# tayloraswift/swift-png

Measured on NVIDIA H100. Metric: MPixels/s decode (inflate+unfilter), higher is better.
Workload: dtype u8

## Files before the change

### swift-png_b200/csrc/inflate_wave.cuh

```cuda
#pragma once

#include "inflate_serial.cuh"

namespace pngb200 {

#ifndef WV_CTAS
#define WV_CTAS 2
#endif
constexpr int      WV_THREADS      = 256;
constexpr int      WV_CTAS_PER_SM  = WV_CTAS;
constexpr int      WV_WARPS        = WV_THREADS / 32;
constexpr uint32_t WV_SUB_BITS     = 256;
constexpr uint32_t WV_BITS         = WV_THREADS * WV_SUB_BITS;
constexpr uint32_t WV_WORDS        = WV_BITS / 32 + 8;
constexpr uint32_t WV_SMEM_WORDS   = WV_WORDS + WV_WORDS / 8 + 1;
constexpr uint32_t WV_RING         = 65536;
constexpr uint32_t WV_WINDOW       = 32768;
constexpr uint32_t WV_OUT_BYTES    = WV_RING - WV_WINDOW;
constexpr uint32_t WV_BITMAP_WORDS = WV_OUT_BYTES / 32;
constexpr uint32_t WV_LIST_CAP     = WV_BITS / 2 + 64;
constexpr uint64_t WV_MAX_WAVE_OUT = (uint64_t)WV_LIST_CAP * 258;
constexpr uint32_t WV_HDR_WORDS    = 192;
constexpr uint32_t ADLER_MOD32     = 65521;
#ifndef WV_POLL_NS
#define WV_POLL_NS 20
#endif
constexpr uint32_t WV_WALK_K       = 8;

#if defined(PNGB200_EMU) && defined(WV_PROFILE)
struct WvProfile { uint64_t thread_iters[8], warp_iters[8]; };
inline WvProfile& wv_profile() { static WvProfile p; return p; }
inline void wv_count(int phase, uint32_t iters)
{
    uint32_t m = iters;
    for (int o = 16; o; o >>= 1) m = max(m, __shfl_xor_sync(0xffffffffu, m, o));
    wv_profile().thread_iters[phase] += iters;
    if ((threadIdx.x & 31) == 0) wv_profile().warp_iters[phase] += m;
}
#define WV_COUNT(phase, iters) wv_count(phase, iters)
#else
#define WV_COUNT(phase, iters)
#endif

enum : uint32_t { PF_EOB = 1, PF_BAD = 2 };
enum : uint32_t { WK_SYNC = 0, WK_END = 1, WK_EOB = 2, WK_BAD = 3, WK_OWN_EOB = 4, WK_OWN_BAD = 5, WK_RUNNING = 6 };

struct WvHeader {
    int32_t  status, type, final, nlit, ndist;
    uint32_t stored;
    uint64_t pos;
};

struct WvShared {
    SerialShared ser;
    uint32_t     words[WV_SMEM_WORDS];
    uint32_t     mask[8 * WV_THREADS];
    uint32_t     ck[8 * WV_THREADS];
    uint32_t     exit_[WV_THREADS];
    uint32_t     wpos_[WV_THREADS];
    uint32_t     wn_[WV_THREADS];
    uint64_t     cross_[WV_THREADS];
    uint16_t     wc_[WV_THREADS];
    uint16_t     next_[WV_THREADS];
    uint8_t      kind_[WV_THREADS];
    uint8_t      wlist[2][WV_THREADS];
    uint16_t     dpre_[WV_THREADS];
    uint16_t     cst_[WV_THREADS];
    uint32_t     dsum[WV_WARPS];
    uint32_t     wcount[3];
    uint32_t     bitmap[WV_BITMAP_WORDS];
    uint8_t      ring[WV_RING] __align__(16);
    uint64_t     warp_sums[WV_WARPS + 1];
    uint32_t     adler_a[WV_WARPS], adler_b[WV_WARPS];
    uint32_t     exc[WV_WARPS], valid[WV_WARPS];
    uint32_t     mark[WV_WARPS];
    uint32_t     last, term, anomaly, ticket;
    uint64_t     cyc[12], tick;
    uint64_t     pf_bar;
    WvHeader     hdr;
};

struct WvParams {
    const StreamJob* jobs;
    StreamResult*    results;
    const uint32_t*  order;
    uint32_t*        ticket;
    uint8_t*         scratch;
    uint64_t         scratch_stride;
    uint64_t         bitmap_words;
    int              count;
    SwitchRecord*    switched = nullptr;
};

struct CopyItem { uint32_t o; uint32_t run_dist; };

#ifdef PNGB200_EMU
typedef uintptr_t saddr_t;
inline uint32_t lds32(saddr_t addr) { return *(const uint32_t*)addr; }
inline uint32_t bfe32(uint32_t x, uint32_t pos, uint32_t len);
inline saddr_t smem_addr(const void* p) { return (uintptr_t)p; }
inline saddr_t opaque(saddr_t a) { return a; }
inline uint32_t bmsk(uint32_t pos, uint32_t width)
{
    pos &= 0xff; width &= 0xff;
    if (pos > 31 || width == 0) return 0;
    const uint32_t m = width >= 32 ? ~0u : (1u << width) - 1u;
    return m << pos;
}
inline uint32_t bfe32(uint32_t x, uint32_t pos, uint32_t len) { return pos > 31 ? 0 : (x >> pos) & bmsk(0, len); }
#else
typedef uint32_t saddr_t;
__device__ __forceinline__ uint32_t lds32(uint32_t addr)
{
    uint32_t v;
    asm volatile("ld.shared.u32 %0, [%1];" : "=r"(v) : "r"(addr) : "memory");
    return v;
}
__device__ __forceinline__ uint32_t bmsk(uint32_t pos, uint32_t width)
{
    uint32_t r;
    asm("bmsk.clamp.b32 %0, %1, %2;" : "=r"(r) : "r"(pos), "r"(width));
    return r;
}
__device__ __forceinline__ uint32_t bfe32(uint32_t x, uint32_t pos, uint32_t len)
{
    return (x >> pos) & bmsk(0, len);
}
__device__ __forceinline__ uint32_t smem_addr(const void* p) { return (uint32_t)__cvta_generic_to_shared(p); }
__device__ __forceinline__ uint32_t opaque(uint32_t a)
{
    asm volatile("" : "+r"(a));
    return a;
}
#endif

#ifdef PNGB200_EMU
inline void mbar_init(uint64_t*, uint32_t) {}
inline void mbar_expect_tx(uint64_t*, uint32_t) {}
inline void bulk_g2s(void* dst, const void* src, uint32_t bytes, uint64_t*) { memcpy(dst, src, bytes); }
inline bool mbar_try_wait(uint64_t*, uint32_t) { return true; }
inline void fence_proxy_async() {}
inline void bulk_prefetch_l2(const void*, uint32_t) {}
#else
__device__ __forceinline__ void mbar_init(uint64_t* bar, uint32_t count)
{
    asm volatile("mbarrier.init.shared::cta.b64 [%0], %1;" ::"r"((uint32_t)__cvta_generic_to_shared(bar)), "r"(count) : "memory");
}
__device__ __forceinline__ void mbar_expect_tx(uint64_t* bar, uint32_t bytes)
{
    asm volatile("mbarrier.arrive.expect_tx.shared::cta.b64 _, [%0], %1;" ::"r"((uint32_t)__cvta_generic_to_shared(bar)), "r"(bytes) : "memory");
}
__device__ __forceinline__ void bulk_g2s(void* dst, const void* src, uint32_t bytes, uint64_t* bar)
{
    asm volatile("cp.async.bulk.shared::cluster.global.mbarrier::complete_tx::bytes [%0], [%1], %2, [%3];" ::"r"(
                     (uint32_t)__cvta_generic_to_shared(dst)),
                 "l"(src), "r"(bytes), "r"((uint32_t)__cvta_generic_to_shared(bar))
                 : "memory");
}
__device__ __forceinline__ bool mbar_try_wait(uint64_t* bar, uint32_t parity)
{
    uint32_t ok;
    asm volatile("{\n\t.reg .pred p;\n\tmbarrier.try_wait.parity.shared::cta.b64 p, [%1], %2;\n\tselp.u32 %0, 1, 0, p;\n\t}"
                 : "=r"(ok)
                 : "r"((uint32_t)__cvta_generic_to_shared(bar)), "r"(parity)
                 : "memory");
    return ok != 0;
}
__device__ __forceinline__ void fence_proxy_async() { asm volatile("fence.proxy.async.shared::cta;" ::: "memory"); }
__device__ __forceinline__ void bulk_prefetch_l2(const void* src, uint32_t bytes)
{
    asm volatile("cp.async.bulk.prefetch.L2.global [%0], %1;" ::"l"(src), "r"(bytes) : "memory");
}
#endif
constexpr uint32_t WV_PF_WORDS = WV_WORDS + 4;

struct FastBits {
    saddr_t  wbase;
    uint32_t wi;
    uint32_t cur, nxt;
    uint32_t off;
    uint32_t pos;
    __device__ __forceinline__ void init(saddr_t words_addr, uint32_t start)
    {
        wbase = words_addr;
        const uint32_t W = start >> 5;
        cur = lds32(wbase + ((W + (W >> 3)) << 2));
        nxt = lds32(wbase + ((W + 1 + ((W + 1) >> 3)) << 2));
        wi  = W + 2;
        off = start & 31;
        pos = start;
    }
    __device__ __forceinline__ uint32_t peek() const { return __funnelshift_r(cur, nxt, off); }
    __device__ __forceinline__ void skip(uint32_t n)
    {
        off += n;
        pos += n;
        if (off >= 32) {
            cur = nxt;
            nxt = lds32(wbase + ((wi + (wi >> 3)) << 2));
            ++wi;
            off -= 32;
        }
    }
};

template <int ROOT>
__device__ __forceinline__ uint32_t fast_lookup(saddr_t table_addr, uint32_t bits)
{
    uint32_t e = lds32(table_addr + ((bits & ((1u << ROOT) - 1u)) << 2));
    if ((e & (E_SPECIAL | E_PTR | E_INVALID)) == (E_SPECIAL | E_PTR))
        e = lds32(table_addr + (((e >> 16) + bfe32(bits, ROOT, e_skip(e) - ROOT)) << 2));
    return e;
}

template <bool WANT_DIST>
__device__ __forceinline__ uint32_t wv_decode(FastBits& b, saddr_t lit, saddr_t dst, uint32_t& run, uint32_t& dist,
                                              uint32_t& is_copy)
{
    const uint32_t bits = b.peek();
    const uint32_t e = fast_lookup<LIT_ROOT>(lit, bits);
    if (e & E_SPECIAL) {
        if (e & E_INVALID) return PF_BAD;
        b.skip(e_len(e));
        return PF_EOB;
    }
    const uint32_t len = e & 15u, skipn = (e >> 4) & 31u;
    run = (e >> 16) + bfe32(bits, len, skipn - len);
    b.skip(skipn);
    is_copy = (e >> 9) & 1u;
    const uint32_t dbits = b.peek();
    const uint32_t d = fast_lookup<DIST_ROOT>(dst, dbits);
    if (is_copy && (d & E_SPECIAL)) return PF_BAD;
    const uint32_t dlen = d & 15u, dskip = (d >> 4) & 31u;
    if (WANT_DIST) dist = (d >> 16) + bfe32(dbits, dlen, dskip - dlen);
    b.skip(is_copy ? dskip : 0u);
    return 0;
}

struct StagedReader {
    const uint32_t* w;
    uint64_t        base_bit, total_bits, pos;
    uint32_t        wi;
    uint64_t        buf;
    int             cnt;
    __device__ void init(const uint32_t* words, uint64_t base, uint64_t total, uint64_t p)
    {
        w = words; base_bit = base; total_bits = total;
        seek(p);
    }
    __device__ void seek(uint64_t p)
    {
        pos = p;
        wi  = (uint32_t)((p - base_bit) >> 5);
        buf = 0;
        cnt = 0;
        refill();
        int skip = (int)(p & 31);
        buf >>= skip;
        cnt -= skip;
    }
    __device__ __forceinline__ void refill()
    {
        while (cnt <= 32) {
            buf |= (uint64_t)(wi < WV_HDR_WORDS ? w[wi] : 0u) << cnt;
            cnt += 32;
            ++wi;
        }
    }
    __device__ __forceinline__ uint32_t peek() const { return (uint32_t)buf; }
    __device__ __forceinline__ void consume(int n) { buf >>= n; cnt -= n; pos += n; }
    __device__ __forceinline__ uint32_t take(int n)
    {
        uint32_t v = (uint32_t)buf & (n >= 32 ? ~0u : ((1u << n) - 1u));
        consume(n);
        return v;
    }
    __device__ __forceinline__ bool have(uint64_t n) const { return pos + n <= total_bits; }
};

__device__ __forceinline__ uint32_t bit_mask(uint32_t lo, uint32_t hi)
{
    return (hi >= 32 ? ~0u : ((1u << hi) - 1u)) & ~((1u << lo) - 1u);
}
__device__ __forceinline__ void bits_set(uint32_t* U, uint32_t o, uint32_t run)
{
    const uint32_t a = o & 31u;
    uint32_t*      w = U + (o >> 5);
    if (a + run <= 32u) { atomicOr(w, bmsk(a, run)); return; }
    atomicOr(w, ~0u << a);
    uint32_t rem = run - (32u - a);
    for (++w; rem >= 32u; ++w, rem -= 32u) atomicOr(w, ~0u);
    if (rem) atomicOr(w, bmsk(0, rem));
}
__device__ __forceinline__ void bits_clear(uint32_t* U, uint32_t o, uint32_t run)
{
    const uint32_t a = o & 31u;
    uint32_t*      w = U + (o >> 5);
    if (a + run <= 32u) { atomicAnd(w, ~bmsk(a, run)); return; }
    atomicAnd(w, ~(~0u << a));
    uint32_t rem = run - (32u - a);
    for (++w; rem >= 32u; ++w, rem -= 32u) atomicAnd(w, 0u);
    if (rem) atomicAnd(w, ~bmsk(0, rem));
}
__device__ __forceinline__ bool bits_all_clear(const uint32_t* U, uint32_t o, uint32_t run)
{
    const volatile uint32_t* w = U + (o >> 5);
    const uint32_t a = o & 31u;
    uint32_t any;
    if (a + run <= 32u) any = *w & bmsk(a, run);
    else {
        any = *w & (~0u << a);
        uint32_t rem = run - (32u - a);
        for (++w; rem >= 32u; ++w, rem -= 32u) any |= *w;
        if (rem) any |= *w & bmsk(0, rem);
    }
    __threadfence_block();
    return any == 0;
}

__device__ __forceinline__ void ring_copy(uint8_t* ring, uint32_t d, uint32_t s, uint32_t run, uint32_t dist)
{
    d &= 0xffffu;
    s &= 0xffffu;
    if (dist >= 4 && max(d, s) + run + 3 < WV_RING) {
        const uint8_t* sp = ring + s;
        uint8_t*       dp = ring + d;
        for (uint32_t k = 0; k < run; k += 4) {
            const uint8_t b0 = sp[k], b1 = sp[k + 1], b2 = sp[k + 2], b3 = sp[k + 3];
            dp[k] = b0;
            if (k + 1 < run) dp[k + 1] = b1;
            if (k + 2 < run) dp[k + 2] = b2;
            if (k + 3 < run) dp[k + 3] = b3;
        }
    } else {
        for (uint32_t k = 0; k < run; ++k) ring[(d + k) & 0xffffu] = ring[(s + k) & 0xffffu];
    }
}

template <typename T>
__device__ __forceinline__ void hbm_copy(T* hbm, uint32_t o, uint32_t run, uint32_t dist)
{
    T*       to   = hbm + o;
    const T* from = to - dist;
    if (dist >= 4) {
        uint32_t k = 0;
        for (; k + 4 <= run; k += 4) {
            const T b0 = from[k], b1 = from[k + 1], b2 = from[k + 2], b3 = from[k + 3];
            to[k] = b0; to[k + 1] = b1; to[k + 2] = b2; to[k + 3] = b3;
        }
        for (; k < run; ++k) to[k] = from[k];
    } else {
        uint32_t q = 0;
        for (uint32_t k = 0; k < run; ++k) {
            to[k] = from[q];
            if (++q == dist) q = 0;
        }
    }
}

struct EmitState {
    uint8_t*  ring;
    uint32_t  rbase;
    uint8_t*  hbm;
    uint32_t* U;
    CopyItem* list;
    uint32_t  reach;
    uint32_t  o;
    uint32_t  first;
    uint32_t  clean;
    uint32_t  c_next;
    bool      bad_ref;
};

template <bool IN_HBM>
__device__ __forceinline__ void emit_token(EmitState& S, uint32_t run, uint32_t dist, uint32_t is_copy)
{
    const uint32_t o = S.o;
    if (!is_copy) {
        if (IN_HBM) S.hbm[o] = (uint8_t)run;
        else S.ring[(S.rbase + o) & 0xffffu] = (uint8_t)run;
        S.o = o + 1;
        return;
    }
    if (dist > S.reach + o) {
        S.bad_ref = true;
        return;
    }
    const int32_t src = (int32_t)o - (int32_t)dist;
    bool final = src + (int32_t)run <= 0 || src >= (int32_t)S.clean;
    if (!final && src >= (int32_t)S.first)
        final = bits_all_clear(S.U, (uint32_t)src, min(run, dist));
    if (final) {
        if (IN_HBM) hbm_copy(S.hbm, o, run, dist);
        else ring_copy(S.ring, S.rbase + o, S.rbase + o - dist, run, dist);
    } else {
        bits_set(S.U, o, run);
        S.list[S.c_next++] = CopyItem{o, run | (dist - 1) << 16};
        S.clean = o + run;
    }
    S.o = o + run;
}

__device__ __forceinline__ void emit_token_sym(EmitState& S, uint32_t run, uint32_t dist, uint32_t is_copy)
{
    uint16_t* const h = reinterpret_cast<uint16_t*>(S.hbm);
    uint32_t o = S.o;
    if (!is_copy) {
        h[o] = (uint16_t)run;
        S.o = o + 1;
        return;
    }
    const uint32_t have = S.reach + o;
    if (dist > have) {
        const uint32_t pre = min(dist - have, run);
        const uint32_t idx = WV_WINDOW - (dist - have);
        for (uint32_t k = 0; k < pre; ++k) h[o + k] = (uint16_t)(0x8000u | (idx + k));
        o += pre;
        run -= pre;
        if (run == 0) { S.o = o; return; }
    }
    const int32_t src = (int32_t)o - (int32_t)dist;
    bool final = src + (int32_t)run <= 0 || src >= (int32_t)S.clean;
    if (!final && src >= (int32_t)S.first) final = bits_all_clear(S.U, (uint32_t)src, min(run, dist));
    if (final) {
        hbm_copy(h, o, run, dist);
    } else {
        bits_set(S.U, o, run);
        S.list[S.c_next++] = CopyItem{o, run | (dist - 1) << 16};
        S.clean = o + run;
    }
    S.o = o + run;
}

template <class Shared>
__device__ bool wv_fast_header(Shared& sh, uint64_t hbase_bit, uint64_t pos, uint64_t total_bits, int lane, WvHeader& out)
{
    const uint32_t* const W = sh.words;
    auto get = [&](uint32_t rel, uint32_t n) -> uint32_t {
        const uint32_t w = rel >> 5;
        const uint32_t v = __funnelshift_r(W[w], W[w + 1], rel & 31u);
        return n >= 32 ? v : v & ((1u << n) - 1u);
    };
    uint32_t rel = (uint32_t)(pos - hbase_bit);
    if (pos + 3 > total_bits) return false;
    const uint32_t h3 = get(rel, 3);
    rel += 3;
    out.status = PNGB200_OK;
    out.final = (int32_t)(h3 & 1u);
    out.type = (int32_t)(h3 >> 1);
    out.stored = 0;
    out.nlit = out.ndist = 0;
    if (out.type == 3) return false;
    if (out.type == 0) {
        const uint64_t boundary = (pos + 3 + 7) & ~(uint64_t)7;
        if (boundary + 32 > total_bits) return false;
        const uint32_t v = get((uint32_t)(boundary - hbase_bit), 32);
        const uint32_t l = v & 0xffffu, m = v >> 16;
        if (l != (~m & 0xffffu)) return false;
        out.stored = l;
        out.pos = boundary + 32;
        return true;
    }
    uint8_t* const lens = sh.ser.lens;
    if (out.type == 1) {
        for (int k = lane; k < 320; k += 32) lens[k] = k < 144 ? 8 : k < 256 ? 9 : k < 280 ? 7 : k < 288 ? 8 : 5;
        out.nlit = 288;
        out.ndist = 32;
        out.pos = pos + 3;
        __syncwarp();
        return true;
    }
    if (pos + 17 > total_bits) return false;
    const uint32_t v = get(rel, 14);
    rel += 14;
    const int nlit = 257 + (int)(v & 31u), ndist = 1 + (int)((v >> 5) & 31u), nclen = 4 + (int)(v >> 10);
    if (nlit > 286) return false;
    if (lane < 19) lens[lane] = 0;
    __syncwarp();
    if (lane < nclen) lens[c_clen_order[lane]] = (uint8_t)get(rel + 3u * (uint32_t)lane, 3);
    rel += 3u * (uint32_t)nclen;
    __syncwarp();
    build_table<META_ROOT, META_CAP>(sh.ser.meta, lens, 19, ALPHA_META, &sh.ser.scratch, lane, 32);
    if (sh.ser.scratch.status) return false;
    __syncwarp();
    uint32_t ok = 1, end_rel = 0;
    if (lane == 0) {
        const uint32_t* const meta = sh.ser.meta;
        uint32_t wi  = rel >> 5;
        uint64_t buf = ((uint64_t)W[wi + 1] << 32 | W[wi]) >> (rel & 31u);
        int      cnt = 64 - (int)(rel & 31u);
        wi += 2;
        const int total = nlit + ndist;
        int       have = 0;
        uint32_t  prev = 0;
        while (have < total) {
            if (cnt < 32) {
                buf |= (uint64_t)(wi < WV_HDR_WORDS ? W[wi] : 0u) << cnt;
                cnt += 32;
                ++wi;
            }
            const uint32_t e = meta[(uint32_t)buf & (META_CAP - 1)];
            if (e & E_SPECIAL) { ok = 0; break; }
            const uint32_t len = e & 15u, sym = e >> 16;
            buf >>= len;
            cnt -= (int)len;
            if (sym < 16) {
                lens[have++] = (uint8_t)sym;
                prev = sym;
                continue;
            }
            uint32_t element, extra, base;
            if (sym == 16) {
                if (have == 0) { ok = 0; break; }
                element = prev; extra = 2; base = 3;
            } else if (sym == 17) {
                element = 0; extra = 3; base = 3;
            } else {
                element = 0; extra = 7; base = 11;
            }
            const int reps = (int)(base + ((uint32_t)buf & ((1u << extra) - 1u)));
            buf >>= extra;
            cnt -= (int)extra;
            if (have + reps > total) { ok = 0; break; }
            for (int k = 0; k < reps; ++k) lens[have + k] = (uint8_t)element;
            prev = element;
            have += reps;
        }
        end_rel = (wi << 5) - (uint32_t)cnt;
    }
    ok = __shfl_sync(0xffffffffu, ok, 0);
    end_rel = __shfl_sync(0xffffffffu, end_rel, 0);
    if (!ok || hbase_bit + end_rel > total_bits) return false;
    out.nlit = nlit;
    out.ndist = ndist;
    out.pos = hbase_bit + end_rel;
    __syncwarp();
    return true;
}

__device__ __forceinline__ void adler_bytes(const uint8_t* p, uint64_t n, uint64_t wt, uint64_t& a, uint64_t& bw)
{
    for (uint64_t i = 0; i < n; ++i) {
        a += p[i];
        bw += (wt - i) * p[i];
    }
}
__device__ __forceinline__ void adler_chunk16_u32(uint4 x, uint32_t wt, uint32_t& a, uint32_t& bw)
{
    const uint32_t s = __vsadu4(x.x, 0) + __vsadu4(x.y, 0) + __vsadu4(x.z, 0) + __vsadu4(x.w, 0);
    const uint32_t wsum = __dp4a(x.x, 0x03020100u, 0u) + __dp4a(x.y, 0x07060504u, 0u) +
                          __dp4a(x.z, 0x0b0a0908u, 0u) + __dp4a(x.w, 0x0f0e0d0cu, 0u);
    a += s;
    bw += wt * s - wsum;
}
__device__ __forceinline__ void adler_chunk16(uint4 x, uint64_t wt, uint64_t& a, uint64_t& bw)
{
    const uint32_t s = __vsadu4(x.x, 0) + __vsadu4(x.y, 0) + __vsadu4(x.z, 0) + __vsadu4(x.w, 0);
    const uint32_t wsum = __dp4a(x.x, 0x03020100u, 0u) + __dp4a(x.y, 0x07060504u, 0u) +
                          __dp4a(x.z, 0x0b0a0908u, 0u) + __dp4a(x.w, 0x0f0e0d0cu, 0u);
    a += s;
    bw += wt * s - wsum;
}

__global__ void __launch_bounds__(WV_THREADS, WV_CTAS_PER_SM) inflate_wave_kernel(WvParams P)
{
    PNGB200_DYN_SMEM(wv_smem);
    WvShared& sh = *reinterpret_cast<WvShared*>(wv_smem);
    const uint32_t t    = threadIdx.x;
    const unsigned lane = lane_id(), warp = t >> 5;
    CopyItem* const list    = reinterpret_cast<CopyItem*>(P.scratch + blockIdx.x * P.scratch_stride);
    uint32_t* const gbitmap = reinterpret_cast<uint32_t*>(P.scratch + blockIdx.x * P.scratch_stride +
                                                         sizeof(CopyItem) * WV_LIST_CAP);
    for (uint32_t k = t; k < WV_BITMAP_WORDS; k += WV_THREADS) sh.bitmap[k] = 0;
    if (t == 0) mbar_init(&sh.pf_bar, 1);
    static_assert(offsetof(WvShared, ck) == offsetof(WvShared, mask) + sizeof(uint32_t) * 8 * WV_THREADS, "prefetch area = mask ++ ck");
    static_assert(sizeof(uint32_t) * WV_PF_WORDS <= 2 * sizeof(uint32_t) * 8 * WV_THREADS && offsetof(WvShared, mask) % 16 == 0, "prefetch area");
    uint32_t pf_parity = 0;
    const saddr_t words_addr = smem_addr(sh.words);
    const saddr_t lit = smem_addr(sh.ser.lit), dstt = smem_addr(sh.ser.dist);
    uint32_t* const mk = sh.mask;

    for (;;) {
        __syncthreads();
        if (t == 0) {
            sh.ticket = atomicAdd(P.ticket, 1u);
            sh.anomaly = 0;
            for (int k = 0; k < 12; ++k) sh.cyc[k] = 0;
            sh.tick = (uint64_t)clock64();
        }
        __syncthreads();
        if (sh.ticket >= (uint32_t)P.count) return;
        const int       j   = P.order ? (int)P.order[sh.ticket] : (int)sh.ticket;
        const StreamJob job = P.jobs[j];
        StreamResult*   r   = P.results + j;

        BitReader br;
        br.init(job.src, job.src_len, job.start_bit);
        uint64_t out    = job.start_out;
        uint32_t blocks = 0, waves = 0, resolve_rounds = 0;
        uint64_t n_tokens = 0, n_matches = 0, n_deferred = 0, walk_tokens = 0;
        int      st     = PNGB200_OK;
        uint32_t phase  = (uint32_t)job.phase;
        uint64_t resume_bit = job.start_bit, resume_out = job.start_out;
        uint8_t* dst     = job.dst;
        uint64_t dst_cap = job.dst_cap;
        bool     sym     = job.symbolic != 0;
        uint32_t esz     = sym ? 2u : 1u;
        uint32_t mis     = (uint32_t)((uintptr_t)dst & 15);
        const bool may_switch = sym && job.may_switch;
        uint64_t   mark_end = 0, sw_out = ~0ull, sw_bytes = 0;
        bool fallback = false, over_cap = false;
        bool ring_stale = job.start_out != 0;
        bool     pf_pending = false;
        uint64_t pf_first = 0;
        const bool adler_on = job.start_out == 0 && !sym;
        uint32_t   s1 = 1, s2 = 0;
        uint64_t   pend_len = 0;
        bool       pend = false;
        auto fold_adler = [&]() {
            if (pend && t == 0) {
                uint64_t A = 0, B = 0;
                for (int w = 0; w < WV_WARPS; ++w) { A += sh.adler_a[w]; B += sh.adler_b[w]; }
                s2 = (uint32_t)((s2 + (pend_len % ADLER_MOD32) * s1 + B) % ADLER_MOD32);
                s1 = (uint32_t)((s1 + A) % ADLER_MOD32);
            }
            pend = false;
        };
        auto adler_hbm = [&](const uint8_t* p, uint64_t n) {
            uint64_t a = 0, bw = 0;
            const uint64_t per = (n + WV_THREADS - 1) / WV_THREADS;
            const uint64_t lo = min((uint64_t)t * per, n), hi = min(lo + per, n);
            adler_bytes(p + lo, hi - lo, n - lo, a, bw);
            uint32_t a32 = (uint32_t)(a % ADLER_MOD32), b32 = (uint32_t)(bw % ADLER_MOD32);
            for (int o = 16; o; o >>= 1) {
                a32 += __shfl_down_sync(0xffffffffu, a32, o);
                b32 += __shfl_down_sync(0xffffffffu, b32, o);
            }
            if (lane == 0) { sh.adler_a[warp] = a32; sh.adler_b[warp] = b32; }
            pend = true;
            pend_len = n;
        };
        auto tick = [&](int i) {
            if (t == 0) {
                const uint64_t now = (uint64_t)clock64();
                sh.cyc[i] += now - sh.tick;
                sh.tick = now;
            }
        };
        auto try_switch = [&]() {
            if (!may_switch || !sym || out < mark_end + WV_WINDOW) return;
            const uint64_t area = (2 * out + 15) & ~(uint64_t)15;
            const uint64_t room = 2 * job.dst_cap;
            if (area + WV_WINDOW > room) return;
            const uint16_t* const s16 = reinterpret_cast<const uint16_t*>(job.dst);
            uint8_t* const        nd  = job.dst + area + WV_WINDOW - out;
            for (uint64_t x = out - WV_WINDOW + t; x < out; x += WV_THREADS) nd[x] = (uint8_t)s16[x];
            __syncthreads();
            sym        = false;
            esz        = 1;
            dst        = nd;
            dst_cap    = room - area - WV_WINDOW + out;
            mis        = (uint32_t)((uintptr_t)nd & 15);
            ring_stale = true;
            sw_out     = out;
            sw_bytes   = area + WV_WINDOW;
        };

        if (phase == 0) {
            st = read_stream_header(br, job.format, r);
            if (st == PNGB200_OK) {
                resume_bit = br.at();
                phase = 1;
            }
        }
        if (st == PNGB200_OK && phase == 2) st = read_trailer(br, job.format, r);

        while (st == PNGB200_OK && phase == 1) {
            __syncthreads();
            fold_adler();
            {
                const uint64_t hbase = br.pos >> 5;
                for (uint32_t k = t; k < WV_HDR_WORDS; k += WV_THREADS) sh.words[k] = br.load_word(hbase + k);
                __syncthreads();
                if (warp == 0) {
                    WvHeader h;
                    if (!wv_fast_header(sh, hbase << 5, br.pos, br.total_bits, (int)lane, h)) {
#ifdef PNGB200_EMU
                        if (lane == 0 && getenv("WV_TRACE_HDR")) fprintf(stderr, "slow header at bit %llu\n", (unsigned long long)br.pos);
#endif
                        int      type0 = 0, final0 = 0, nlit0 = 0, ndist0 = 0;
                        uint32_t stored0 = 0;
                        StagedReader sr;
                        sr.init(sh.words, hbase << 5, br.total_bits, br.pos);
                        int st0 = parse_block_header(sr, &sh.ser, r, (int)lane, &type0, &final0, &stored0, &nlit0, &ndist0);
                        h = WvHeader{st0, type0, final0, nlit0, ndist0, stored0, sr.pos};
                    }
                    if (lane == 0) sh.hdr = h;
                }
            }
            __syncthreads();
            const WvHeader hdr = sh.hdr;
            st = hdr.status;
            if (st != PNGB200_OK) break;
            const int      type = hdr.type, final = hdr.final;
            const uint32_t stored = hdr.stored;
            br.seek(hdr.pos);
            if (type != 0) {
                st = build_block_tables(&sh.ser, r, hdr.nlit, hdr.ndist, (int)t, WV_THREADS);
                if (st != PNGB200_OK) break;
            }
            tick(0);
            if (type == 0) {
                if (!br.have(8 * (uint64_t)stored)) { st = PNGB200_NEED_MORE_INPUT; break; }
                if (out + stored > dst_cap) { st = fail(r, PNGB200_ERR_OUTPUT_CAPACITY); break; }
                const uint8_t* s = job.src + (br.at() >> 3);
                if (sym) for (uint32_t k = t; k < stored; k += WV_THREADS) reinterpret_cast<uint16_t*>(dst)[out + k] = s[k];
                else for (uint32_t k = t; k < stored; k += WV_THREADS) dst[out + k] = s[k];
                if (adler_on && stored) adler_hbm(s, stored);
                if (stored) ring_stale = true;
                out += stored;
                br.seek(br.pos + 8 * (uint64_t)stored);
                __syncthreads();
                fold_adler();
                try_switch();
                tick(9);
            } else {
                bool block_done = false;
                while (!block_done) {
                    ++waves;
                    const uint64_t wstart = br.pos;
                    const uint64_t wbase  = (wstart >> 5) & ~(uint64_t)7;
                    __syncthreads();
                    bool staged = false;
                    if (pf_pending) {
                        while (!mbar_try_wait(&sh.pf_bar, pf_parity)) {}
                        pf_parity ^= 1;
                        pf_pending = false;
                        if (wbase >= pf_first && wbase - pf_first < 4) {
                            const uint32_t* lin = sh.mask + (uint32_t)(wbase - pf_first);
                            for (uint32_t k = t; k < WV_WORDS; k += WV_THREADS) sh.words[k + (k >> 3)] = lin[k];
                            staged = true;
                        }
                    }
                    if (!staged)
                        for (uint32_t k = t; k < WV_WORDS; k += WV_THREADS)
                            sh.words[k + (k >> 3)] = br.load_word(wbase + k);
                    if (t == 0) sh.wcount[0] = 0;
                    __syncthreads();
                    fold_adler();
                    tick(1);
                    const uint32_t rel0  = (uint32_t)(wstart - (wbase << 5));
                    const uint32_t base  = t * WV_SUB_BITS;
                    const uint32_t limit = base + WV_SUB_BITS;

                    uint32_t nout = 0, ncopy = 0, flags = 0, exit_bit;
                    {
#pragma unroll
                        for (int k = 0; k < 8; ++k) mk[k * WV_THREADS + t] = 0;
                        sh.ck[t] = 0;
                        FastBits b;
                        b.init(words_addr, t == 0 ? rel0 : base);
                        uint32_t mi = 0, mw = 0, n = 0;
                        while (b.pos < limit) {
                            const uint32_t rr = b.pos - base, wi = rr >> 5;
                            if (wi != mi) {
                                mk[mi * WV_THREADS + t] = mw;
                                mw = 0;
                                mi = wi;
                                sh.ck[wi * WV_THREADS + t] = nout | ncopy << 16;
                            }
                            mw |= 1u << (rr & 31);
                            uint32_t run = 0, dist = 0, cp = 0;
                            const uint32_t s = wv_decode<false>(b, lit, dstt, run, dist, cp);
                            if (s) { flags = s; break; }
                            nout += cp ? run : 1u;
                            ncopy += cp;
                            ++n;
                        }
                        mk[mi * WV_THREADS + t] = mw;
                        exit_bit = b.pos;
                        WV_COUNT(0, n);
                    }
                    sh.exit_[t] = exit_bit;
                    sh.cross_[t] = 0;
                    __syncthreads();
                    tick(2);

                    {
                        uint32_t u = t, pos = exit_bit, wn = 0, wc = 0;
                        bool     active = flags == 0;
                        if (!active) {
                            sh.kind_[t] = (uint8_t)(flags == PF_EOB ? WK_OWN_EOB : WK_OWN_BAD);
                            sh.wpos_[t] = exit_bit;
                            sh.wn_[t] = 0;
                            sh.wc_[t] = 0;
                        }
                        for (uint32_t round = 0;; ++round) {
                            const uint32_t K = WV_WALK_K << min(round, 6u);
                            bool     still = false;
                            uint32_t iters = 0;
                            if (active) {
                                FastBits b;
                                b.init(words_addr, pos);
                                uint32_t kind = WK_RUNNING;
                                const uint32_t first_sub = sh.exit_[u] >> 8;
                                bool     crossed = sh.cross_[u] != 0;
                                for (; iters < K; ++iters) {
                                    const uint32_t p = b.pos;
                                    if (p >= WV_BITS) { kind = WK_END; break; }
                                    const uint32_t s = p >> 8, rr = p & 255u;
                                    if (!crossed && s > first_sub) {
                                        sh.cross_[u] = 1ull << 63 | (uint64_t)p << 40 | (uint64_t)(wc & 0xffu) << 24 | (wn & 0xffffffu);
                                        crossed = true;
                                    }
                                    if ((mk[(rr >> 5) * WV_THREADS + s] >> (rr & 31)) & 1u) { kind = WK_SYNC; break; }
                                    uint32_t run = 0, dist = 0, cp = 0;
                                    const uint32_t e = wv_decode<false>(b, lit, dstt, run, dist, cp);
                                    if (e) { kind = e == PF_EOB ? WK_EOB : WK_BAD; break; }
                                    wn += cp ? run : 1u;
                                    wc += cp;
                                }
                                sh.wpos_[u] = b.pos;
                                sh.wn_[u]   = wn;
                                sh.wc_[u]   = (uint16_t)wc;
                                sh.kind_[u] = (uint8_t)kind;
                                still = kind == WK_RUNNING;
                                walk_tokens += iters;
                            }
                            WV_COUNT(1, iters);
                            if (t == 0) sh.wcount[(round + 1) % 3] = 0;
                            const unsigned bal = __ballot_sync(0xffffffffu, still);
                            if (still) {
                                uint32_t at = 0;
                                const int leader = __ffs((int)bal) - 1;
                                if ((int)lane == leader) at = atomicAdd(&sh.wcount[round % 3], (uint32_t)__popc(bal));
                                at = __shfl_sync(bal, at, leader);
                                sh.wlist[round & 1][at + __popc(bal & ((1u << lane) - 1u))] = (uint8_t)u;
                            }
                            __syncthreads();
                            const uint32_t cnt = sh.wcount[round % 3];
                            if (cnt == 0) break;
                            active = t < cnt;
                            if (active) {
                                u   = sh.wlist[round & 1][t];
                                pos = sh.wpos_[u];
                                wn  = sh.wn_[u];
                                wc  = sh.wc_[u];
                            }
                        }
                    }
                    tick(3);
                    const uint32_t kind = sh.kind_[t], wpos = sh.wpos_[t];
                    {
                        const bool joins_next = kind == WK_SYNC && (wpos >> 8) == t + 1;
                        sh.next_[t] = (uint16_t)(kind == WK_SYNC ? wpos >> 8 : 0xffffu);
                        const unsigned e = __ballot_sync(0xffffffffu, !joins_next);
                        if (lane == 0) sh.exc[warp] = e;
                    }
                    __syncthreads();

                    if (t == 0) {
                        uint32_t E[WV_WARPS];
#pragma unroll
                        for (int w = 0; w < WV_WARPS; ++w) E[w] = sh.exc[w];
                        uint32_t cur = 0, x = 0;
                        bool     done = false;
#pragma unroll
                        for (int w = 0; w < WV_WARPS; ++w) {
                            uint32_t v = 0;
                            while (!done && cur < 32u * (w + 1)) {
                                const uint32_t lo = cur - 32u * w;
                                const uint32_t m = E[w] & (~0u << lo);
                                if (m == 0) {
                                    v |= ~0u << lo;
                                    cur = 32u * (w + 1);
                                    break;
                                }
                                const uint32_t b = (uint32_t)__ffs((int)m) - 1;
                                x = 32u * w + b;
                                v |= bit_mask(lo, b + 1);
                                const uint32_t nx = sh.next_[x];
                                if (nx == 0xffffu) done = true;
                                else cur = nx;
                            }
                            sh.valid[w] = v;
                        }
                        sh.last = x;
                        sh.term = sh.kind_[x];
                    }
                    __syncthreads();
                    tick(4);

                    const bool     on_chain = (sh.valid[warp] >> lane) & 1u;
                    const uint32_t last = sh.last, term = sh.term;
                    uint32_t from = rel0, to = exit_bit;
                    uint32_t my_nout = 0, my_ncopy = 0;
                    bool     adopted = false;
                    if (on_chain) {
                        uint32_t pn = 0, pc = 0, pre_n = 0, pre_c = 0;
                        if (t > 0) {
                            uint32_t w = warp, m = sh.valid[w] & ((1u << lane) - 1u);
                            while (m == 0) m = sh.valid[--w];
                            const uint32_t pred = w * 32 + 31 - (uint32_t)__clz((int)m);
                            const uint32_t p0 = sh.wpos_[pred];
                            from = sh.exit_[pred];
                            pn = sh.wn_[pred];
                            pc = sh.wc_[pred];
                            if (pred + 1 < t) {
                                const uint64_t cr = sh.cross_[pred];
                                if (cr) {
                                    from = (uint32_t)(cr >> 40) & 0x1ffffu;
                                    pn -= (uint32_t)cr & 0xffffffu;
                                    pc -= (uint32_t)(cr >> 24) & 0xffu;
                                }
                            }
                            const uint32_t rr = p0 - base, q = rr >> 5;
                            const uint32_t ck = sh.ck[q * WV_THREADS + t];
                            pre_n = ck & 0xffffu;
                            pre_c = ck >> 16;
                            const uint32_t first = (uint32_t)__ffs((int)mk[q * WV_THREADS + t]) - 1;
                            if (first != (rr & 31)) {
                                FastBits b;
                                b.init(words_addr, base + 32 * q + first);
                                while (b.pos != p0 && b.pos < limit) {
                                    uint32_t run = 0, dist = 0, cp = 0;
                                    if (wv_decode<false>(b, lit, dstt, run, dist, cp)) break;
                                    pre_n += cp ? run : 1u;
                                    pre_c += cp;
                                }
                            }
                        }
                        my_nout  = pn + nout - pre_n;
                        my_ncopy = pc + ncopy - pre_c;
                        if (t == last) {
                            to = wpos;
                            my_nout += sh.wn_[t];
                            my_ncopy += sh.wc_[t];
                            if (term == WK_BAD || term == WK_OWN_BAD || (wbase << 5) + wpos > br.total_bits)
                                sh.anomaly = 1;
                        }
                    }
                    else if (t > 0 && ((sh.valid[(t - 1) >> 5] >> ((t - 1) & 31)) & 1u) && sh.kind_[t - 1] == WK_SYNC) {
                        const uint64_t cr = sh.cross_[t - 1];
                        if (cr) {
                            adopted  = true;
                            from     = sh.exit_[t - 1];
                            to       = (uint32_t)(cr >> 40) & 0x1ffffu;
                            my_nout  = (uint32_t)cr & 0xffffffu;
                            my_ncopy = (uint32_t)(cr >> 24) & 0xffu;
                        }
                    }
                    const uint64_t mine = (uint64_t)my_ncopy << 40 | my_nout;
                    uint64_t incl = mine;
                    for (int o = 1; o < 32; o <<= 1) {
                        uint64_t v = __shfl_up_sync(0xffffffffu, incl, o);
                        if ((int)lane >= o) incl += v;
                    }
                    if (lane == 31) sh.warp_sums[warp] = incl;
                    __syncthreads();
                    if (warp == 0) {
                        uint64_t ws = lane < WV_WARPS ? sh.warp_sums[lane] : 0, wi = ws;
                        for (int o = 1; o < 32; o <<= 1) {
                            uint64_t v = __shfl_up_sync(0xffffffffu, wi, o);
                            if ((int)lane >= o) wi += v;
                        }
                        if (lane < WV_WARPS) sh.warp_sums[lane] = wi - ws;
                        if (lane == WV_WARPS - 1) sh.warp_sums[WV_WARPS] = wi;
                    }
                    __syncthreads();
                    tick(5);
                    const uint64_t excl    = sh.warp_sums[warp] + incl - mine;
                    const uint32_t o_start = (uint32_t)(excl & 0xffffffffffull);
                    const uint32_t c_start = (uint32_t)(excl >> 40);
                    const uint64_t total64 = sh.warp_sums[WV_WARPS] & 0xffffffffffull;
                    const uint32_t np      = (uint32_t)(sh.warp_sums[WV_WARPS] >> 40);
                    if (sh.anomaly || out + total64 > dst_cap || total64 > P.bitmap_words * 32) {
                        fallback = true;
                        over_cap = out + total64 > dst_cap;
                        break;
                    }
                    const uint32_t  total  = (uint32_t)total64;
                    {
                        const uint64_t nbase = wbase + WV_BITS / 32;
                        const uint64_t first = nbase - ((((uintptr_t)br.words >> 2) + nbase) & 3);
                        if (first >= 1 && (first + WV_PF_WORDS + 1) * 32 <= br.total_bits) {
                            if (t == 0) {
                                fence_proxy_async();
                                mbar_expect_tx(&sh.pf_bar, sizeof(uint32_t) * WV_PF_WORDS);
                                bulk_g2s(sh.mask, br.words + first, sizeof(uint32_t) * WV_PF_WORDS, &sh.pf_bar);
                            }
                            pf_pending = true;
                            pf_first = first;
                        }
                    }
                    uint8_t* const  wdst   = dst + out * esz;
                    const bool      in_hbm = sym || total > WV_OUT_BYTES;
                    const uint32_t  rbase  = (uint32_t)(out + mis) & 0xffffu;
                    uint32_t* const U      = total > WV_OUT_BYTES ? gbitmap : sh.bitmap;
                    if (!in_hbm && ring_stale) {
                        const uint64_t lo = out > WV_WINDOW ? out - WV_WINDOW : 0;
                        for (uint64_t x = lo + t; x < out; x += WV_THREADS) sh.ring[(x + mis) & 0xffffu] = dst[x];
                        __syncthreads();
                    }
                    ring_stale = in_hbm;
                    uint32_t deferred = 0, emitted = 0;
                    if (on_chain || adopted) {
                        EmitState S;
                        S.ring = sh.ring; S.rbase = rbase; S.hbm = wdst; S.U = U; S.list = list;
                        S.reach = out >= WV_WINDOW ? 0x7fffffffu : (uint32_t)out;
                        S.o = o_start; S.first = o_start; S.clean = o_start; S.c_next = c_start;
                        S.bad_ref = false;
                        FastBits b;
                        b.init(words_addr, from);
                        if (sym) {
                            while (b.pos != to && b.pos < WV_BITS + 64) {
                                uint32_t run = 0, dist = 0, cp = 0;
                                if (wv_decode<true>(b, lit, dstt, run, dist, cp)) break;
                                emit_token_sym(S, run, dist, cp);
                                ++emitted;
                            }
                        } else if (in_hbm) {
                            while (b.pos != to && b.pos < WV_BITS + 64) {
                                uint32_t run = 0, dist = 0, cp = 0;
                                if (wv_decode<true>(b, lit, dstt, run, dist, cp)) break;
                                emit_token<true>(S, run, dist, cp);
                                ++emitted;
                            }
                        } else {
                            while (b.pos != to && b.pos < WV_BITS + 64) {
                                uint32_t run = 0, dist = 0, cp = 0;
                                if (wv_decode<true>(b, lit, dstt, run, dist, cp)) break;
                                emit_token<false>(S, run, dist, cp);
                                ++emitted;
                            }
                        }
                        if (S.bad_ref) sh.anomaly = 1;
                        deferred = S.c_next - c_start;
                    }
                    WV_COUNT(2, emitted);
                    uint32_t dincl = deferred;
                    for (int o = 1; o < 32; o <<= 1) {
                        const uint32_t v = __shfl_up_sync(0xffffffffu, dincl, o);
                        if ((int)lane >= o) dincl += v;
                    }
                    if (lane == 31) sh.dsum[warp] = dincl;
                    __threadfence_block();
                    __syncthreads();
                    tick(6);
                    uint32_t nd = 0;
                    {
                        uint32_t below = 0;
#pragma unroll
                        for (int w = 0; w < WV_WARPS; ++w) {
                            const uint32_t v = sh.dsum[w];
                            below += w < (int)warp ? v : 0u;
                            nd += v;
                        }
                        sh.dpre_[t] = (uint16_t)(below + dincl - deferred);
                        sh.cst_[t]  = (uint16_t)c_start;
                    }
                    __syncthreads();
                    if (!sh.anomaly && nd) {
                        auto slot_of = [&](uint32_t g) -> uint32_t {
                            uint32_t lo = 0, hi = WV_THREADS;
                            while (hi - lo > 1) {
                                const uint32_t mid = (lo + hi) >> 1;
                                if (sh.dpre_[mid] <= g) lo = mid;
                                else hi = mid;
                            }
                            return (uint32_t)sh.cst_[lo] + g - sh.dpre_[lo];
                        };
                        uint32_t g = t, rounds = 0;
                        CopyItem it = CopyItem{0, 0}, n1 = it, n2 = it;
                        if (g < nd) it = list[slot_of(g)];
                        if (g + WV_THREADS < nd) n1 = list[slot_of(g + WV_THREADS)];
                        if (g + 2 * WV_THREADS < nd) n2 = list[slot_of(g + 2 * WV_THREADS)];
                        for (;;) {
                            bool progressed = false;
                            if (g < nd) {
                                const uint32_t run = it.run_dist & 0xffff, dist = (it.run_dist >> 16) + 1;
                                const int32_t  src = (int32_t)it.o - (int32_t)dist;
                                const int32_t  hi  = src + (int32_t)min(run, dist);
                                bool ready = true;
                                if (hi > 0) {
                                    const uint32_t lo = (uint32_t)max(src, 0);
                                    ready = bits_all_clear(U, lo, (uint32_t)hi - lo);
                                }
                                if (ready) {
                                    if (sym) hbm_copy(reinterpret_cast<uint16_t*>(wdst), it.o, run, dist);
                                    else if (in_hbm) hbm_copy(wdst, it.o, run, dist);
                                    else ring_copy(sh.ring, rbase + it.o, rbase + it.o - dist, run, dist);
                                    __threadfence_block();
                                    bits_clear(U, it.o, run);
                                    g += WV_THREADS;
                                    it = n1;
                                    n1 = n2;
                                    if (g + 2 * WV_THREADS < nd) n2 = list[slot_of(g + 2 * WV_THREADS)];
                                    progressed = true;
                                }
                            }
                            ++rounds;
                            if (!__any_sync(0xffffffffu, g < nd)) break;
                            if (!__any_sync(0xffffffffu, progressed)) __nanosleep(WV_POLL_NS);
                        }
                        resolve_rounds += rounds;
                        WV_COUNT(4, rounds);
                    }
                    __threadfence_block();
                    __syncthreads();
                    tick(7);
                    if (sh.anomaly) {
                        for (uint32_t k = t; k < (total + 31) / 32; k += WV_THREADS) U[k] = 0;
                        fallback = true;
                        break;
                    }
                    if (may_switch && sym) {
                        const uint16_t* const ws = reinterpret_cast<const uint16_t*>(wdst);
                        uint32_t lm = 0;
                        for (uint32_t k = t; k < total; k += WV_THREADS)
                            if (ws[k] & 0x8000u) lm = k + 1;
                        for (int o = 16; o; o >>= 1) lm = max(lm, __shfl_xor_sync(0xffffffffu, lm, o));
                        if (lane == 0) sh.mark[warp] = lm;
                        __syncthreads();
                        uint32_t wm = 0;
#pragma unroll
                        for (int w = 0; w < WV_WARPS; ++w) wm = max(wm, sh.mark[w]);
                        if (wm) mark_end = out + wm;
                    }
                    if (!in_hbm && total) {
                        const uint32_t shift = rbase & 15u;
                        uint8_t* const gbase = wdst - shift;
                        const uint32_t rb16  = rbase - shift;
                        const uint32_t end   = shift + total;
                        const uint32_t nq    = (end + 15) >> 4;
                        uint32_t a = 0, bw = 0;
                        for (uint32_t c = t; c < nq; c += WV_THREADS) {
                            const uint32_t lo = c << 4, hi = lo + 16;
                            if (lo >= shift && hi <= end) {
                                const uint4 x = *reinterpret_cast<const uint4*>(sh.ring + ((rb16 + lo) & 0xffffu));
                                reinterpret_cast<uint4*>(gbase)[c] = x;
                                adler_chunk16_u32(x, end - lo, a, bw);
                            } else {
                                for (uint32_t k = max(lo, shift); k < min(hi, end); ++k) {
                                    const uint8_t v = sh.ring[(rb16 + k) & 0xffffu];
                                    gbase[k] = v;
                                    a += v;
                                    bw += (end - k) * v;
                                }
                            }
                        }
                        if (adler_on) {
                            uint32_t a32 = a, b32 = bw % ADLER_MOD32;
                            for (int o = 16; o; o >>= 1) {
                                a32 += __shfl_down_sync(0xffffffffu, a32, o);
                                b32 += __shfl_down_sync(0xffffffffu, b32, o);
                            }
                            if (lane == 0) { sh.adler_a[warp] = a32; sh.adler_b[warp] = b32; }
                            pend = true;
                            pend_len = total;
                        }
                    } else if (in_hbm && adler_on) {
                        adler_hbm(wdst, total);
                    }
                    tick(8);
                    out += total;
                    if (t == 0) n_matches += np;
                    n_tokens += emitted;
                    n_deferred += deferred;
                    br.seek((wbase << 5) + sh.wpos_[last]);
                    if (term == WK_EOB || term == WK_OWN_EOB) block_done = true;
                    try_switch();
                }
                if (fallback) break;
            }
            ++blocks;
            resume_bit = br.at();
            resume_out = out;
            if (job.stop_bit && !final && br.at() >= job.stop_bit) break;
            if (final) {
                phase = 2;
                st = read_trailer(br, job.format, r);
                break;
            }
        }
        if (pf_pending) {
            while (!mbar_try_wait(&sh.pf_bar, pf_parity)) {}
            pf_parity ^= 1;
            pf_pending = false;
        }
        __syncthreads();
        fold_adler();
        __syncthreads();
        {
            uint64_t v0 = n_tokens, v1 = n_deferred, v2 = walk_tokens;
            uint32_t v3 = resolve_rounds;
            for (int o = 16; o; o >>= 1) {
                v0 += __shfl_down_sync(0xffffffffu, v0, o);
                v1 += __shfl_down_sync(0xffffffffu, v1, o);
                v2 += __shfl_down_sync(0xffffffffu, v2, o);
                v3 = max(v3, __shfl_down_sync(0xffffffffu, v3, o));
            }
            if (lane == 0) {
                sh.warp_sums[warp] = v0;
                sh.adler_a[warp] = (uint32_t)min(v1, (uint64_t)0xffffffffu);
                sh.adler_b[warp] = (uint32_t)min(v2, (uint64_t)0xffffffffu);
                sh.exc[warp] = v3;
            }
            __syncthreads();
            if (t == 0) {
                uint64_t tk = 0, df = 0, wt = 0;
                uint32_t rr = 0;
                for (int w = 0; w < WV_WARPS; ++w) {
                    tk += sh.warp_sums[w];
                    df += sh.adler_a[w];
                    wt += sh.adler_b[w];
                    rr = max(rr, sh.exc[w]);
                }
                r->stat_waves          = waves;
                r->stat_sync_rounds    = (uint32_t)min(wt, (uint64_t)0xffffffffu);
                r->stat_resolve_rounds = rr;
                r->stat_tokens         = tk;
                r->stat_matches        = n_matches;
                r->stat_deferred       = df;
                for (int k = 0; k < 12; ++k) r->stat_cycles[k] = sh.cyc[k];
            }
        }
        if (fallback && job.symbolic) {
            if (t == 0) {
                r->status = sw_out != ~0ull && over_cap ? PNGB200_ERR_OUTPUT_CAPACITY : PNGB200_ERR_INTERNAL;
                r->produced = out;
                r->consumed_bits = br.at();
                r->blocks = blocks;
            }
        } else if (fallback) {
            __syncthreads();
            if (warp == 0) serial_inflate(sh.ser, job, r, resume_bit, resume_out, 1, blocks);
        } else if (t == 0) {
            if (r->status == 0) r->status = st;
            r->produced      = out;
            r->consumed_bits = br.at();
            r->blocks        = blocks;
            r->resume_bit    = resume_bit;
            r->resume_out    = resume_out;
            r->phase         = phase;
            if (adler_on && job.format != PNGB200_FORMAT_GZIP) {
                const uint32_t computed = s2 << 16 | s1;
                r->checksum = computed;
                r->ck_done  = 1;
                if (r->trailer_seen && job.format != PNGB200_FORMAT_IOS && r->status >= 0 && r->declared != computed) {
                    r->status = PNGB200_ERR_STREAM_CHECKSUM;
                    r->err_a  = r->declared;
                    r->err_b  = computed;
                }
            }
        }
        if (t == 0) r->stat_fallback = fallback ? 1u : 0u;
        if (t == 0 && may_switch && P.switched) P.switched[j] = SwitchRecord{sw_out != ~0ull ? sw_out : out, sw_bytes};
    }
}

#ifndef PNGB200_EMU
inline int configure_inflate_wave()
{
    return (int)cudaFuncSetAttribute(inflate_wave_kernel, cudaFuncAttributeMaxDynamicSharedMemorySize,
                                     (int)sizeof(WvShared));
}
#endif

inline uint64_t wv_bitmap_words(uint64_t max_dst_cap)
{
    uint64_t bytes = max_dst_cap < WV_MAX_WAVE_OUT ? max_dst_cap : WV_MAX_WAVE_OUT;
    return (bytes + 31) / 32 + 8;
}
inline uint64_t wv_scratch_stride(uint64_t bitmap_words)
{
    uint64_t s = sizeof(CopyItem) * (uint64_t)WV_LIST_CAP + 4 * bitmap_words;
    return (s + 255) / 256 * 256;
}

}
```

Before: 10530.

## Overlap next block header parse with deferred copy resolution in last warp

When a wave ends at a non-final block's end-of-block and output stays in the shared-memory ring, the last warp parses the next deflate block header and issues its bulk prefetch while the other warps resolve the deferred back-reference copies. The copy loop strides by 224 threads instead of 256 in that case. The next loop iteration skips the serial header load and parse if the pre-parsed header is valid. This hides header-parsing latency, but the copy phase loses one warp, and the prefetch barrier parity handling becomes more complex.

Result: faster. 10730, median of 6 (+1.8%).

```diff
diff --git a/swift-png_b200/csrc/inflate_wave.cuh b/swift-png_b200/csrc/inflate_wave.cuh
--- a/swift-png_b200/csrc/inflate_wave.cuh
+++ b/swift-png_b200/csrc/inflate_wave.cuh
@@ -78,6 +78,7 @@
     uint64_t     cyc[12], tick;
     uint64_t     pf_bar;
     WvHeader     hdr;
+    uint32_t     hdr_ready;
 };
 
 struct WvParams {
@@ -585,6 +586,7 @@
         if (t == 0) {
             sh.ticket = atomicAdd(P.ticket, 1u);
             sh.anomaly = 0;
+            sh.hdr_ready = 0;
             for (int k = 0; k < 12; ++k) sh.cyc[k] = 0;
             sh.tick = (uint64_t)clock64();
         }
@@ -613,6 +615,15 @@
         bool ring_stale = job.start_out != 0;
         bool     pf_pending = false;
         uint64_t pf_first = 0;
+        auto pf_start = [&](uint64_t nbase) -> uint64_t {
+            const uint64_t first = nbase - ((((uintptr_t)br.words >> 2) + nbase) & 3);
+            return first >= 1 && (first + WV_PF_WORDS + 1) * 32 <= br.total_bits ? first : 0;
+        };
+        auto pf_issue = [&](uint64_t first) {
+            fence_proxy_async();
+            mbar_expect_tx(&sh.pf_bar, sizeof(uint32_t) * WV_PF_WORDS);
+            bulk_g2s(sh.mask, br.words + first, sizeof(uint32_t) * WV_PF_WORDS, &sh.pf_bar);
+        };
         const bool adler_on = job.start_out == 0 && !sym;
         uint32_t   s1 = 1, s2 = 0;
         uint64_t   pend_len = 0;
@@ -678,7 +689,8 @@
         while (st == PNGB200_OK && phase == 1) {
             __syncthreads();
             fold_adler();
-            {
+            const bool preparsed = sh.hdr_ready != 0;
+            if (!preparsed) {
                 const uint64_t hbase = br.pos >> 5;
                 for (uint32_t k = t; k < WV_HDR_WORDS; k += WV_THREADS) sh.words[k] = br.load_word(hbase + k);
                 __syncthreads();
@@ -709,6 +721,7 @@
                 st = build_block_tables(&sh.ser, r, hdr.nlit, hdr.ndist, (int)t, WV_THREADS);
                 if (st != PNGB200_OK) break;
             }
+            if (t == 0) sh.hdr_ready = 0;
             tick(0);
             if (type == 0) {
                 if (!br.have(8 * (uint64_t)stored)) { st = PNGB200_NEED_MORE_INPUT; break; }
@@ -980,18 +993,10 @@
                         break;
                     }
                     const uint32_t  total  = (uint32_t)total64;
-                    {
-                        const uint64_t nbase = wbase + WV_BITS / 32;
-                        const uint64_t first = nbase - ((((uintptr_t)br.words >> 2) + nbase) & 3);
-                        if (first >= 1 && (first + WV_PF_WORDS + 1) * 32 <= br.total_bits) {
-                            if (t == 0) {
-                                fence_proxy_async();
-                                mbar_expect_tx(&sh.pf_bar, sizeof(uint32_t) * WV_PF_WORDS);
-                                bulk_g2s(sh.mask, br.words + first, sizeof(uint32_t) * WV_PF_WORDS, &sh.pf_bar);
-                            }
-                            pf_pending = true;
-                            pf_first = first;
-                        }
+                    if (const uint64_t first = pf_start(wbase + WV_BITS / 32)) {
+                        if (t == 0) pf_issue(first);
+                        pf_pending = true;
+                        pf_first = first;
                     }
                     uint8_t* const  wdst   = dst + out * esz;
                     const bool      in_hbm = sym || total > WV_OUT_BYTES;
@@ -1060,7 +1065,30 @@
                         sh.cst_[t]  = (uint16_t)c_start;
                     }
                     __syncthreads();
-                    if (!sh.anomaly && nd) {
+                    const uint64_t next_bit = (wbase << 5) + sh.wpos_[last];
+                    const bool overlap = (term == WK_EOB || term == WK_OWN_EOB) && !final && !in_hbm && !sh.anomaly &&
+                                         !(job.stop_bit && next_bit - br.lead_bits >= job.stop_bit);
+                    const uint32_t nt = overlap ? WV_THREADS - 32 : WV_THREADS;
+                    const bool hdr_warp = overlap && warp == WV_WARPS - 1;
+                    if (hdr_warp) {
+                        const uint64_t hbase = next_bit >> 5;
+                        for (uint32_t k = lane; k < WV_HDR_WORDS; k += 32) sh.words[k] = br.load_word(hbase + k);
+                        __syncwarp();
+                        WvHeader h;
+                        bool ok = wv_fast_header(sh, hbase << 5, next_bit, br.total_bits, (int)lane, h);
+                        if (lane == 0) {
+                            if (ok && h.type != 0) {
+                                if (pf_pending) while (!mbar_try_wait(&sh.pf_bar, pf_parity)) {}
+                                if (const uint64_t first = pf_start((h.pos >> 5) & ~(uint64_t)7)) pf_issue(first);
+                            }
+#if defined(PNGB200_EMU) && defined(WV_PROFILE)
+                            wv_profile().thread_iters[ok ? 5 : 6] += 1;
+#endif
+                            sh.hdr = h;
+                            sh.hdr_ready = ok;
+                        }
+                    }
+                    if (!hdr_warp && !sh.anomaly && nd) {
                         auto slot_of = [&](uint32_t g) -> uint32_t {
                             uint32_t lo = 0, hi = WV_THREADS;
                             while (hi - lo > 1) {
@@ -1073,8 +1101,8 @@
                         uint32_t g = t, rounds = 0;
                         CopyItem it = CopyItem{0, 0}, n1 = it, n2 = it;
                         if (g < nd) it = list[slot_of(g)];
-                        if (g + WV_THREADS < nd) n1 = list[slot_of(g + WV_THREADS)];
-                        if (g + 2 * WV_THREADS < nd) n2 = list[slot_of(g + 2 * WV_THREADS)];
+                        if (g + nt < nd) n1 = list[slot_of(g + nt)];
+                        if (g + 2 * nt < nd) n2 = list[slot_of(g + 2 * nt)];
                         for (;;) {
                             bool progressed = false;
                             if (g < nd) {
@@ -1092,10 +1120,10 @@
                                     else ring_copy(sh.ring, rbase + it.o, rbase + it.o - dist, run, dist);
                                     __threadfence_block();
                                     bits_clear(U, it.o, run);
-                                    g += WV_THREADS;
+                                    g += nt;
                                     it = n1;
                                     n1 = n2;
-                                    if (g + 2 * WV_THREADS < nd) n2 = list[slot_of(g + 2 * WV_THREADS)];
+                                    if (g + 2 * nt < nd) n2 = list[slot_of(g + 2 * nt)];
                                     progressed = true;
                                 }
                             }
@@ -1107,8 +1135,15 @@
                         WV_COUNT(4, rounds);
                     }
                     __threadfence_block();
+                    if (overlap) tick(7);
                     __syncthreads();
-                    tick(7);
+                    tick(overlap ? 0 : 7);
+                    if (overlap && sh.hdr_ready && sh.hdr.type != 0) {
+                        if (pf_pending) pf_parity ^= 1;
+                        const uint64_t first = pf_start((sh.hdr.pos >> 5) & ~(uint64_t)7);
+                        pf_pending = first != 0;
+                        pf_first = first;
+                    }
                     if (sh.anomaly) {
                         for (uint32_t k = t; k < (total + 31) / 32; k += WV_THREADS) U[k] = 0;
                         fallback = true;
```
